# Nobita421/signature-Gan

Measured on AMD Instinct MI355X. Metric: signature images/sec (G+D train step, bs64 64x64 z=100), higher is better.
Workload: dtype f32; 1 GPU; configs[1]: reference conv G/D 64x64x1, z=100, batch 64 per GPU, f32, n_critic=1; global_batch=64, parallelism=dp1

## Files before the change

### include/siggan.h

```cpp
#ifndef SIGGAN_H
#define SIGGAN_H

#include <stddef.h>
#include <stdint.h>

#ifdef __cplusplus
extern "C" {
#endif

#define SIGGAN_ABI_VERSION 4

enum {
    SIGGAN_OK = 0,
    SIGGAN_E_INVALID = -1,
    SIGGAN_E_STATE = -2,
    SIGGAN_E_HIP = -3,
    SIGGAN_E_NOMEM = -4
};

typedef struct siggan_ctx siggan_ctx;

typedef struct siggan_config {
    int32_t device;
    int32_t latent_dim;
// ... 2 lines not shown
    int32_t max_batch;
    float   dropout;
    float   leaky_slope;
    uint64_t seed;
    int32_t dtype;
    float   f16_grad_scale;
    int32_t spectral_norm;
    float   g_leaky_slope;
} siggan_config;
enum { SIGGAN_DTYPE_F32 = 0, SIGGAN_DTYPE_BF16 = 1, SIGGAN_DTYPE_F16 = 2 };

typedef struct siggan_storage {
    float *g_params, *g_grads, *g_exp_avg, *g_exp_avg_sq, *g_adam_steps;
    float *g_bn_running_mean, *g_bn_running_var;
    int64_t *g_bn_batches;
    float *d_params, *d_grads, *d_exp_avg, *d_exp_avg_sq, *d_adam_steps;
    float *d_sn_u, *d_sn_v;
} siggan_storage;

typedef struct siggan_hyper {
    double lr, beta1, beta2, eps;
    float label_smoothing;
    float clip_max_norm;
    float grad_scale;
} siggan_hyper;

enum {
    SIGGAN_M_D_LOSS = 0, SIGGAN_M_D_LOSS_REAL, SIGGAN_M_D_LOSS_FAKE, SIGGAN_M_D_REAL_MEAN,
    SIGGAN_M_D_FAKE_MEAN, SIGGAN_M_D_REAL_ACC, SIGGAN_M_D_FAKE_ACC, SIGGAN_M_D_GRAD_NORM,
    SIGGAN_M_G_LOSS, SIGGAN_M_G_FAKE_MEAN, SIGGAN_M_G_GRAD_NORM,
    SIGGAN_M_D_SKIPPED, SIGGAN_M_G_SKIPPED,
    SIGGAN_M_COUNT = 16
};

int siggan_abi_version(void);
const char *siggan_last_error(void);
int siggan_create(const siggan_config *cfg, siggan_ctx **out);
int siggan_destroy(siggan_ctx *ctx);

int64_t siggan_param_count(const siggan_ctx *ctx, int which);
int32_t siggan_param_tensors(const siggan_ctx *ctx, int which);
int siggan_param_span(const siggan_ctx *ctx, int which, int32_t idx, int64_t *offset, int64_t *numel);
int64_t siggan_bn_count(const siggan_ctx *ctx);
int64_t siggan_sn_count(const siggan_ctx *ctx, int which);
int32_t siggan_bn_layers(const siggan_ctx *ctx);
int64_t siggan_workspace_bytes(const siggan_ctx *ctx);

int siggan_bind(siggan_ctx *ctx, const siggan_storage *st);
int siggan_params_changed(siggan_ctx *ctx);
int siggan_seed(siggan_ctx *ctx, uint64_t seed, uint64_t offset);
int siggan_rng_state(siggan_ctx *ctx, uint64_t *seed, uint64_t *offset);
#define SIGGAN_MODE_GRAPH 1
#define SIGGAN_MODE_OVERLAP 2
int siggan_set_mode(siggan_ctx *ctx, int32_t mode);

enum { SIGGAN_STEP_TRAINER = 0, SIGGAN_STEP_ABLATION = 1 };
int siggan_set_step_variant(siggan_ctx *ctx, int32_t variant);

int siggan_g_forward(siggan_ctx *ctx, const float *z_dev, int32_t batch, int32_t training,
                     float *images_dev, void *stream);

enum { SIGGAN_IS_NEG = 0, SIGGAN_IS_INK_SIGNED = 1, SIGGAN_IS_INK_UNIT = 2, SIGGAN_IS_COUNT = 3 };
int siggan_g_generate_u8(siggan_ctx *ctx, const float *z_dev, int32_t batch, uint8_t *u8_dev,
                         float *images_dev, int32_t *stats_dev, float threshold, void *stream);

int siggan_g_latent_grad(siggan_ctx *ctx, const float *z_dev, int32_t batch, const uint8_t *target_u8_dev,
                         const float *target_f32_dev, float *dz_dev, float *loss_dev, float *images_dev, void *stream);

typedef struct siggan_latent_objective {
    float recon_weight;
    float realism_weight;
    float prior_weight;
} siggan_latent_objective;

int siggan_g_latent_objective_grad(siggan_ctx *ctx, const float *z_dev, int32_t batch, const uint8_t *target_u8_dev,
                                   const float *target_f32_dev, const siggan_latent_objective *w, float *dz_dev,
                                   float *objective_dev, float *terms_dev, float *probs_dev, float *images_dev, void *stream);

int siggan_g_latent_objective_grad_seeded(siggan_ctx *ctx, const float *z_dev, int32_t batch, const uint8_t *target_u8_dev,
        const float *target_f32_dev, const siggan_latent_objective *w, const float *image_grad_dev, float *dz_dev,
        float *objective_dev, float *terms_dev, float *probs_dev, float *images_dev, void *stream);

int siggan_g_param_grad(siggan_ctx *ctx, const float *z_dev, int32_t batch, const uint8_t *target_u8_dev,
                        const float *target_f32_dev, const siggan_latent_objective *w, int32_t first_layer,
                        float *dparams_dev, float *objective_dev, float *terms_dev, float *probs_dev, float *images_dev,
                        void *stream);

int siggan_d_forward(siggan_ctx *ctx, const float *x_dev, int32_t batch, int32_t training,
                     const float *masks_dev, float *probs_dev, float *features_dev, void *stream);

int siggan_d_score_u8(siggan_ctx *ctx, const uint8_t *u8_dev, int32_t batch, int32_t binarize, float *probs_dev,
                      float *x_dev, void *stream);
int siggan_dequant_table(float *table_host);

int siggan_d_step(siggan_ctx *ctx, const float *real_dev, int32_t batch, const float *z_dev,
                  const float *masks_dev, const siggan_hyper *hp, float *metrics_dev,
                  float *metrics_host, void *stream);
int siggan_g_step(siggan_ctx *ctx, int32_t batch, const float *z_dev, const siggan_hyper *hp,
                  float *metrics_dev, float *metrics_host, void *stream);

#define SIGGAN_COMM_ID_BYTES 128
int siggan_comm_unique_id(void *id_out);
int siggan_comm_init(siggan_ctx *ctx, int32_t rank, int32_t world, const void *id);
int siggan_comm_destroy(siggan_ctx *ctx);
int32_t siggan_comm_world(const siggan_ctx *ctx);
int siggan_comm_broadcast(siggan_ctx *ctx, void *buf_dev, int64_t bytes, int32_t root, void *stream);
// ... 45 lines not shown
```

### signature-gan_amd/csrc/gconv.h

```cpp
#pragma once
#include <hip/hip_runtime.h>
#include <stdint.h>
#include <vector>

#include "act.h"

namespace siggan {

enum Epilogue : int {
    EPI_RAW = 0,
    EPI_BIAS_LRELU_DROP,
    EPI_AFFINE_RELU,
    EPI_LRELU_BWD,
    EPI_BN_BWD_STATS,
};

struct GConvArgs {
    int dt;
    const void* in;
    const void* wp;
    void* out;
    int B, Hi, Wi, Ci, Co;
    int lgHr, lgWr;
    int Ho, Wo;
    int form;
    int M;
    int epi;
    const float* bias;
    const float* noise;
    const float* scale;
    const float* shift;
    const void* aref;
    const float* bnp;
    float* stat0;
    float* stat1;
    int64_t stat_cap;
    const float* cls_w;
    float* cls_part;
    float slope;
    float gslope;
    float* slab;
    int64_t slab_floats;
    size_t slab_stride;
    const float* zeros;
};

struct BnBwdParams { f32x4 sc, sf, mu, rs; };
__device__ __forceinline__ BnBwdParams bn_bwd_params(const float* __restrict__ bnp, int Co, int co) {
    BnBwdParams q;
    q.sc = *reinterpret_cast<const f32x4*>(bnp + co); q.sf = *reinterpret_cast<const f32x4*>(bnp + Co + co);
    q.mu = *reinterpret_cast<const f32x4*>(bnp + 2 * Co + co); q.rs = *reinterpret_cast<const f32x4*>(bnp + 3 * Co + co);
    return q;
}
template <class T, bool LK>
__device__ __forceinline__ void bn_bwd_stat_terms(const f32x4 v, const f32x4 y, const BnBwdParams& q, float gs, f32x4& s0, f32x4& s1) {
#pragma unroll
    for (int e = 0; e < 4; ++e) {
        const float vq = (float)(T)v[e];
        const float d = g_dact<LK>(fmaf(y[e], q.sc[e], q.sf[e]), vq, gs);
        s0[e] += d;
        s1[e] = fmaf(d, (y[e] - q.mu[e]) * q.rs[e], s1[e]);
    }
}
__host__ __device__ inline bool gen_lk(const GConvArgs& a) {
    return a.gslope != 0.f && (a.epi == EPI_AFFINE_RELU || a.epi == EPI_BN_BWD_STATS);
}

struct WgradArgs {
    int dt;
    const void* S;
    const void* L;
    float* slab;
    float* dw;
    float* db;
    int B, Cs, Cl;
    int lgHs, lgWs, lgCl;
    int K;
    int kchunk;
    const float* zeros;
};

struct Prof {
    struct Rec {
        int id; double flops, bytes; hipEvent_t e0, e1;
        int form, epi_req, epi, M, Ci, Co;
    };
    static constexpr int NID = 8;
    std::vector<Rec> recs;
    static const char* name(int id);
    void begin(int id, double flops, double bytes, hipStream_t st);
    void shape(const GConvArgs& a, int epi_req);
    void clear();
};
extern Prof* g_prof;

int launch_gconv(const GConvArgs& a, hipStream_t st);
void launch_gconv16(int cfg, const GConvArgs& a, dim3 grid, hipStream_t st, hipEvent_t e0, hipEvent_t e1, int kq = 1);
void launch_wgrad16(bool small, const WgradArgs& a, dim3 grid, hipStream_t st, hipEvent_t e0, hipEvent_t e1);
int launch_wgrad(WgradArgs a, int max_splits, hipStream_t st);

}
```

### signature-gan_amd/csrc/gconv.hip

```cpp
#include "gconv.h"
#include <hip/hip_ext.h>

namespace siggan {


static constexpr int BK = 32;
static constexpr int PAD = 4;

__device__ __forceinline__ int xcd_remap(int bid, int nwg) {
    const int q = nwg >> 3, r = nwg & 7, xcd = bid & 7, idx = bid >> 3;
    return (xcd < r ? xcd * (q + 1) : r * (q + 1) + (xcd - r) * q) + idx;
}

template <int BM, int BN, int WM, int WN, int BK = 32, int DEEP = 0, int KQ = 1, bool LK = false>
__global__ __launch_bounds__(256 * KQ) void k_gconv(const GConvArgs a) {
    constexpr int TM = BM / (32 * WM), TN = BN / (32 * WN);
    constexpr int PA = BM / 32, PB = BN / 32;
    constexpr int KC = BK / 32;
    constexpr int LD = BK + 4;
    __shared__ __attribute__((aligned(16))) float smem[KQ * 2 * LD * (BM + BN)];
    const int quad = KQ > 1 ? (int)(threadIdx.x >> 8) : 0;
    float* const sA = smem + quad * (2 * LD * (BM + BN));
    float* const sB = sA + 2 * LD * BM;

    const int tid = threadIdx.x & 255, lane = tid & 63, wave = tid >> 6;
    const int li = lane & 31, lh = lane >> 5;
    const int wm = wave / WN, wn = wave % WN;
    const float* const a_in = static_cast<const float*>(a.in);
    const float* const a_wp = static_cast<const float*>(a.wp);

    const int tiles_n = a.Co / BN;
    const int bid = xcd_remap(blockIdx.x, gridDim.x);
    const int m0 = (bid / tiles_n) * BM, n0 = (bid % tiles_n) * BN;
    const int cls = blockIdx.z, ph = cls >> 1, pw = cls & 1;
    const int Hr = 1 << a.lgHr, Wr = 1 << a.lgWr;
    const int ntaps = a.form == 0 ? 16 : 4;
    const int Ktot = ntaps * a.Ci;
    const int lgcpt = 31 - __builtin_clz(a.Ci / BK);
    const int nk_all = ntaps << lgcpt;
    const int kper = (nk_all + gridDim.y * KQ - 1) / (gridDim.y * KQ);
    const int k_lo = (blockIdx.y * KQ + quad) * kper;
    const int k_hi = min(nk_all, k_lo + kper);
    const int nk = k_hi - k_lo;

    const int kc = tid & 7, rloc = tid >> 3;
    const float* a_base[PA];
    int a_ih0[PA], a_iw0[PA];
#pragma unroll
    for (int p = 0; p < PA; ++p) {
        const int m = m0 + rloc + 32 * p;
        if (m < a.M) {
            const int n = m >> (a.lgHr + a.lgWr);
            const int rh = (m >> a.lgWr) & (Hr - 1), rw = m & (Wr - 1);
            a_base[p] = a_in + (size_t)n * a.Hi * a.Wi * a.Ci + kc * 4;
            if (a.form == 0) { a_ih0[p] = 2 * rh - 1; a_iw0[p] = 2 * rw - 1; }
            else             { a_ih0[p] = rh + ph;    a_iw0[p] = rw + pw; }
        } else {
            a_base[p] = a_in; a_ih0[p] = -(1 << 20); a_iw0[p] = -(1 << 20);
        }
    }
    const float* wcur = a_wp + ((size_t)cls * a.Co + n0 + rloc) * Ktot + kc * 4 + (size_t)k_lo * BK;

    const float* a_cur[PA];
    int a_step[PA];
    int l_tap = k_lo >> lgcpt, l_cc = k_lo & ((1 << lgcpt) - 1);
    auto set_tap = [&]() __attribute__((always_inline)) {
        int dh, dw;
        if (a.form == 0) { dh = l_tap >> 2; dw = l_tap & 3; } else { dh = -(l_tap >> 1); dw = -(l_tap & 1); }
#pragma unroll
        for (int p = 0; p < PA; ++p) {
            const int ih = a_ih0[p] + dh, iw = a_iw0[p] + dw;
            const bool ok = (unsigned)ih < (unsigned)a.Hi && (unsigned)iw < (unsigned)a.Wi;
            a_cur[p] = ok ? a_base[p] + ((size_t)(ih * a.Wi + iw) * a.Ci + l_cc * BK) : a.zeros;
            a_step[p] = ok ? BK : 0;
        }
    };
    constexpr int NSET = DEEP ? 2 : 1;
    f32x4 ra[NSET][PA][KC], rb[NSET][PB][KC];
    auto load_tile = [&](int set = 0) __attribute__((always_inline)) {
#pragma unroll
        for (int p = 0; p < PA; ++p) {
#pragma unroll
            for (int q = 0; q < KC; ++q) ra[set][p][q] = *reinterpret_cast<const f32x4*>(a_cur[p] + 32 * q);
            a_cur[p] += a_step[p];
        }
#pragma unroll
        for (int p = 0; p < PB; ++p)
#pragma unroll
            for (int q = 0; q < KC; ++q) rb[set][p][q] = *reinterpret_cast<const f32x4*>(wcur + (size_t)(32 * p) * Ktot + 32 * q);
        wcur += BK;
        if (++l_cc == (1 << lgcpt)) { l_cc = 0; ++l_tap; set_tap(); }
    };
    auto store_tile = [&](int buf, int set = 0) __attribute__((always_inline)) {
        float* dA = sA + buf * LD * BM + rloc * LD + kc * 4;
        float* dB = sB + buf * LD * BN + rloc * LD + kc * 4;
#pragma unroll
        for (int p = 0; p < PA; ++p)
#pragma unroll
            for (int q = 0; q < KC; ++q) *reinterpret_cast<f32x4*>(dA + 32 * p * LD + 32 * q) = ra[set][p][q];
#pragma unroll
        for (int p = 0; p < PB; ++p)
#pragma unroll
            for (int q = 0; q < KC; ++q) *reinterpret_cast<f32x4*>(dB + 32 * p * LD + 32 * q) = rb[set][p][q];
    };

    f32x16 acc[TM][TN];
#pragma unroll
    for (int i = 0; i < TM; ++i)
#pragma unroll
        for (int j = 0; j < TN; ++j)
#pragma unroll
            for (int r = 0; r < 16; ++r) acc[i][j][r] = 0.f;

    if (DEEP && nk >= 5) {
        auto tile = [&](const int h, const int kt, const bool st, const bool ld) __attribute__((always_inline)) {
            const float* pA = sA + h * LD * BM + (wm * (32 * TM) + li) * LD + 4 * lh;
            const float* pB = sB + h * LD * BN + (wn * (32 * TN) + li) * LD + 4 * lh;
            f32x4 fa[2][TM], fb[2][TN];
#pragma unroll
            for (int i = 0; i < TM; ++i) fa[0][i] = *reinterpret_cast<const f32x4*>(pA + 32 * i * LD);
#pragma unroll
            for (int j = 0; j < TN; ++j) fb[0][j] = *reinterpret_cast<const f32x4*>(pB + 32 * j * LD);
#pragma unroll
            for (int c = 0; c < BK / 8; ++c) {
                const int cur = c & 1, nxt = cur ^ 1;
                if (c + 1 < BK / 8) {
#pragma unroll
                    for (int i = 0; i < TM; ++i) fa[nxt][i] = *reinterpret_cast<const f32x4*>(pA + 32 * i * LD + 8 * (c + 1));
#pragma unroll
                    for (int j = 0; j < TN; ++j) fb[nxt][j] = *reinterpret_cast<const f32x4*>(pB + 32 * j * LD + 8 * (c + 1));
                }
                __builtin_amdgcn_sched_barrier(0);
#pragma unroll
                for (int t = 0; t < 4; ++t)
#pragma unroll
                    for (int i = 0; i < TM; ++i)
#pragma unroll
                        for (int j = 0; j < TN; ++j)
                            acc[i][j] = __builtin_amdgcn_mfma_f32_32x32x2f32(fa[cur][i][t], fb[cur][j][t], acc[i][j], 0, 0, 0);
                if (c == 0 && st) store_tile(h ^ 1, h ^ 1);
                if (c == 1 && ld) load_tile(h ^ 1);
            }
            __syncthreads();
        };
        set_tap();
        load_tile(0);
        load_tile(1);
        store_tile(0, 0);
        load_tile(0);
        __syncthreads();
        int kt = 0;
        for (; kt + 4 < nk; kt += 2) {
            tile(0, kt, true, true);
            tile(1, kt + 1, true, true);
        }
        for (; kt < nk; kt += 2) {
            tile(0, kt, kt + 1 < nk, kt + 3 < nk);
            if (kt + 1 < nk) tile(1, kt + 1, kt + 2 < nk, kt + 4 < nk);
        }
    } else {
    if (nk > 0) {
        set_tap();
        load_tile();
        store_tile(0);
        if (nk > 1) load_tile();
    }
    __syncthreads();

    for (int kt = 0; kt < nk; ++kt) {
        const int buf = kt & 1;
        const float* pA = sA + buf * LD * BM + (wm * (32 * TM) + li) * LD + 4 * lh;
        const float* pB = sB + buf * LD * BN + (wn * (32 * TN) + li) * LD + 4 * lh;
        f32x4 fa[2][TM], fb[2][TN];
#pragma unroll
        for (int i = 0; i < TM; ++i) fa[0][i] = *reinterpret_cast<const f32x4*>(pA + 32 * i * LD);
#pragma unroll
        for (int j = 0; j < TN; ++j) fb[0][j] = *reinterpret_cast<const f32x4*>(pB + 32 * j * LD);
#pragma unroll
        for (int c = 0; c < BK / 8; ++c) {
            const int cur = c & 1, nxt = cur ^ 1;
            if (c + 1 < BK / 8) {
#pragma unroll
                for (int i = 0; i < TM; ++i) fa[nxt][i] = *reinterpret_cast<const f32x4*>(pA + 32 * i * LD + 8 * (c + 1));
#pragma unroll
                for (int j = 0; j < TN; ++j) fb[nxt][j] = *reinterpret_cast<const f32x4*>(pB + 32 * j * LD + 8 * (c + 1));
            }
            __builtin_amdgcn_sched_barrier(0);
#pragma unroll
            for (int t = 0; t < 4; ++t)
#pragma unroll
                for (int i = 0; i < TM; ++i)
#pragma unroll
                    for (int j = 0; j < TN; ++j)
                        acc[i][j] = __builtin_amdgcn_mfma_f32_32x32x2f32(fa[cur][i][t], fb[cur][j][t], acc[i][j], 0, 0, 0);
            if (c == 0 && kt + 1 < nk) store_tile(buf ^ 1);
            if (c == 1 && kt + 2 < nk) load_tile();
        }
        __syncthreads();
    }
    }

    float* const outp = gridDim.y > 1 ? a.slab + (size_t)blockIdx.y * a.slab_stride : static_cast<float*>(a.out);
    const int epi = gridDim.y > 1 ? (int)EPI_RAW : a.epi;
    constexpr int LDT = BN + 4;
    static_assert(BM * LDT <= 2 * LD * (BM + BN), "output tile must fit the staging buffers");
    float* const sT = smem;
    if (KQ > 1) {
        float* const red = smem + 2 * LD * (BM + BN);
        if (quad == 1) {
#pragma unroll
            for (int i = 0; i < TM; ++i)
#pragma unroll
                for (int j = 0; j < TN; ++j)
#pragma unroll
                    for (int r = 0; r < 16; ++r) red[(((wave * TM + i) * TN + j) * 16 + r) * 64 + lane] = acc[i][j][r];
        }
        __syncthreads();
        if (quad == 0) {
#pragma unroll
            for (int i = 0; i < TM; ++i)
#pragma unroll
                for (int j = 0; j < TN; ++j)
#pragma unroll
                    for (int r = 0; r < 16; ++r) acc[i][j][r] += red[(((wave * TM + i) * TN + j) * 16 + r) * 64 + lane];
        }
    }
    if (quad == 0) {
#pragma unroll
        for (int i = 0; i < TM; ++i)
#pragma unroll
            for (int j = 0; j < TN; ++j)
#pragma unroll
                for (int r = 0; r < 16; ++r)
                    sT[(wm * (32 * TM) + 32 * i + (r & 3) + 8 * (r >> 2) + 4 * lh) * LDT + wn * (32 * TN) + 32 * j + li] = acc[i][j][r];
    }
    __syncthreads();
    if (quad != 0 && epi != EPI_BN_BWD_STATS) return;
    constexpr int C4 = BN / 4, RPP = 256 / C4;
    const int c4 = tid % C4, r0 = tid / C4;
    const int co = n0 + c4 * 4;
    BnBwdParams bq;
    f32x4 st0 = {0.f, 0.f, 0.f, 0.f}, st1 = st0;
    if (epi == EPI_BN_BWD_STATS) bq = bn_bwd_params(a.bnp, a.Co, co);
    const f32x4 bias4 = epi == EPI_BIAS_LRELU_DROP ? *reinterpret_cast<const f32x4*>(a.bias + co) : f32x4{0.f, 0.f, 0.f, 0.f};
    f32x4 sc4 = {1.f, 1.f, 1.f, 1.f}, sh4 = {0.f, 0.f, 0.f, 0.f};
    if (epi == EPI_AFFINE_RELU) { sc4 = *reinterpret_cast<const f32x4*>(a.scale + co); sh4 = *reinterpret_cast<const f32x4*>(a.shift + co); }
    const bool use_noise = (epi == EPI_BIAS_LRELU_DROP || epi == EPI_LRELU_BWD) && a.noise != nullptr;
#pragma unroll
    for (int p = 0; p < BM / RPP; ++p) {
        const int row = r0 + RPP * p, m = m0 + row;
        if (m >= a.M || quad != 0) continue;
        const int n = m >> (a.lgHr + a.lgWr);
        size_t opix;
        if (a.form == 0) {
            opix = (size_t)m;
        } else {
            const int rh = (m >> a.lgWr) & (Hr - 1), rw = m & (Wr - 1);
            opix = ((size_t)n * a.Ho + 2 * rh + ph) * a.Wo + 2 * rw + pw;
        }
        const size_t o = opix * a.Co + co;
        f32x4 v = *reinterpret_cast<const f32x4*>(sT + row * LDT + c4 * 4);
        if (epi == EPI_BN_BWD_STATS) {
            bn_bwd_stat_terms<float, LK>(v, *reinterpret_cast<const f32x4*>(static_cast<const float*>(a.aref) + o), bq, a.gslope, st0, st1);
        } else if (epi == EPI_BIAS_LRELU_DROP) {
#pragma unroll
            for (int e = 0; e < 4; ++e) { float t = v[e] + bias4[e]; v[e] = t > 0.f ? t : t * a.slope; }
            if (use_noise) {
                const f32x4 nz = *reinterpret_cast<const f32x4*>(a.noise + (size_t)n * a.Co + co);
#pragma unroll
                for (int e = 0; e < 4; ++e) v[e] *= nz[e];
            }
        } else if (epi == EPI_AFFINE_RELU) {
#pragma unroll
            for (int e = 0; e < 4; ++e) v[e] = g_act<LK>(fmaf(v[e], sc4[e], sh4[e]), a.gslope);
        } else if (epi == EPI_LRELU_BWD) {
            const f32x4 ar = *reinterpret_cast<const f32x4*>(static_cast<const float*>(a.aref) + o);
#pragma unroll
            for (int e = 0; e < 4; ++e) v[e] *= ar[e] > 0.f ? 1.f : a.slope;
            if (use_noise) {
                const f32x4 nz = *reinterpret_cast<const f32x4*>(a.noise + (size_t)n * a.Co + co);
#pragma unroll
                for (int e = 0; e < 4; ++e) v[e] *= nz[e];
            }
        }
        *reinterpret_cast<f32x4*>(outp + o) = v;
    }
    if (epi == EPI_BN_BWD_STATS) {
        __syncthreads();
        if (quad == 0) {
            *reinterpret_cast<f32x4*>(sT + (size_t)tid * 8) = st0;
            *reinterpret_cast<f32x4*>(sT + (size_t)tid * 8 + 4) = st1;
// ... 172 lines not shown
    if (i >= total4) return;
    const float4* sl = reinterpret_cast<const float4*>(a.slab);
    const size_t stride4 = a.slab_stride / 4;
    float4 v = sl[i];
    for (int z = 1; z < nsplit; ++z) {
        const float4 w = sl[(size_t)z * stride4 + i];
        v.x += w.x; v.y += w.y; v.z += w.z; v.w += w.w;
    }
    const int C4 = a.Co / 4;
    const int64_t per_img = (int64_t)C4 * a.Ho * a.Wo;
    const bool p2 = (C4 & (C4 - 1)) == 0 && (per_img & (per_img - 1)) == 0;
    const int c = (p2 ? (int)(i & (C4 - 1)) : (int)(i % C4)) * 4;
    const int64_t n = p2 ? i >> (63 - __builtin_clzll(per_img)) : i / per_img;
    float* e = reinterpret_cast<float*>(&v);
    if (a.epi == EPI_BIAS_LRELU_DROP) {
#pragma unroll
        for (int k = 0; k < 4; ++k) {
            float x = e[k] + a.bias[c + k];
            x = x > 0.f ? x : x * a.slope;
            if (a.noise) x *= a.noise[n * a.Co + c + k];
            e[k] = x;
        }
    } else if (a.epi == EPI_AFFINE_RELU) {
#pragma unroll
        for (int k = 0; k < 4; ++k) e[k] = g_act<LK>(fmaf(e[k], a.scale[c + k], a.shift[c + k]), a.gslope);
    } else if (a.epi == EPI_LRELU_BWD) {
        const f32x4 ar = ld4<T>(static_cast<const T*>(a.aref) + i * 4);
        const float* r = reinterpret_cast<const float*>(&ar);
#pragma unroll
        for (int k = 0; k < 4; ++k) {
            float x = e[k] * (r[k] > 0.f ? 1.f : a.slope);
            if (a.noise) x *= a.noise[n * a.Co + c + k];
            e[k] = x;
        }
    }
    st4<T>(static_cast<T*>(a.out) + i * 4, f32x4{v.x, v.y, v.z, v.w});
    if (a.cls_w) {
        __shared__ float shc[4];
        const f32x4 w4 = *reinterpret_cast<const f32x4*>(a.cls_w + (size_t)(p2 ? (i & (per_img - 1)) : (i % per_img)) * 4);
        float d = (float)(T)v.x * w4[0];
        d = fmaf((float)(T)v.y, w4[1], d); d = fmaf((float)(T)v.z, w4[2], d); d = fmaf((float)(T)v.w, w4[3], d);
#pragma unroll
        for (int o = 32; o > 0; o >>= 1) d += __shfl_down(d, o, 64);
        if ((threadIdx.x & 63) == 0) shc[threadIdx.x >> 6] = d;
        __syncthreads();
        if (threadIdx.x == 0) a.cls_part[blockIdx.x] = ((shc[0] + shc[1]) + shc[2]) + shc[3];
    }
}

Prof* g_prof = nullptr;

const char* Prof::name(int id) {
    static const char* n[NID] = {"k_gconv<128,128>", "k_gconv<128,64>", "k_gconv<64,64>", "k_gconv<128,32>",
                                 "k_wgrad<64,64>", "k_gconv_up4", "k_wgrad<32,128>", "?"};
    return n[id < 0 || id >= NID ? NID - 1 : id];
}
void Prof::begin(int id, double flops, double bytes, hipStream_t) {
    Rec r; r.id = id; r.flops = flops; r.bytes = bytes;
    r.form = r.epi_req = r.epi = r.M = r.Ci = r.Co = -1;
    (void)hipEventCreate(&r.e0); (void)hipEventCreate(&r.e1);
    recs.push_back(r);
}
void Prof::shape(const GConvArgs& a, int epi_req) {
    Rec& r = recs.back();
    r.form = a.form; r.epi_req = epi_req; r.epi = a.epi; r.M = a.M; r.Ci = a.Ci; r.Co = a.Co;
}
void Prof::clear() {
    for (auto& r : recs) { (void)hipEventDestroy(r.e0); (void)hipEventDestroy(r.e1); }
    recs.clear();
}

static double gconv_bytes(const GConvArgs& a) {
    const double es = (double)dt_size(a.dt);
    const double in = (double)a.B * a.Hi * a.Wi * a.Ci, out = (double)a.B * a.Ho * a.Wo * a.Co, w = 16.0 * a.Ci * a.Co;
    return es * (in + w + out * (a.epi == EPI_LRELU_BWD ? 2.0 : 1.0));
}
static double wgrad_bytes(const WgradArgs& a) {
    const double es = (double)dt_size(a.dt);
    return es * ((double)a.K * a.Cs + 4.0 * a.K * a.Cl) + 4.0 * 16.0 * a.Cs * a.Cl;
}

template <int BM, int BN, int WM, int WN, int BKT = 32, int DEEP = 0, int KQ = 1>
static int launch_cfg(const GConvArgs& a_in, hipStream_t st, int id, int nsplit) {
    GConvArgs a = a_in;
    const int tiles = ((a.M + BM - 1) / BM) * (a.Co / BN);
    const int ncls = a.form == 0 ? 1 : 4;
    const int64_t total4 = (int64_t)a.B * a.Ho * a.Wo * a.Co / 4;
    int rows = 0;
    if (a.epi == EPI_BN_BWD_STATS) {
        if (nsplit > 1 && (256 % (a.Co / 4)) != 0) nsplit = 1;
        rows = nsplit > 1 ? (int)((total4 + 255) / 256) : ((a.M + BM - 1) / BM) * ncls;
        if ((int64_t)2 * rows * a.Co > a.stat_cap) { a.epi = EPI_RAW; rows = 0; }
        else a.stat1 = a.stat0 + (size_t)rows * a.Co;
    }
    if (a.cls_w) {
        const int64_t per_img4 = (int64_t)a.Ho * a.Wo * a.Co / 4;
        if (nsplit > 1 && a.epi != EPI_BN_BWD_STATS && total4 % 256 == 0 && per_img4 % 256 == 0) rows = (int)(per_img4 / 256);
        else a.cls_w = nullptr;
    }
    dim3 grid(tiles, nsplit, ncls);
    if (g_prof) {
        g_prof->begin(id, 2.0 * a.M * a.Co * (double)((a.form == 0 ? 16 : 4) * a.Ci) * ncls, gconv_bytes(a), st);
        g_prof->shape(a, a_in.epi);
    }
    hipEvent_t e0 = g_prof ? g_prof->recs.back().e0 : nullptr, e1 = g_prof ? g_prof->recs.back().e1 : nullptr;
    if (a.dt != DT_F32) {
        launch_gconv16(id, a, grid, st, e0, e1, KQ);
    } else if (gen_lk(a)) {
        hipExtLaunchKernelGGL((k_gconv<BM, BN, WM, WN, BKT, DEEP, KQ, true>), grid, dim3(256 * KQ), 0, st, e0, e1, 0, a);
    } else if (g_prof) {
        hipExtLaunchKernelGGL((k_gconv<BM, BN, WM, WN, BKT, DEEP, KQ>), grid, dim3(256 * KQ), 0, st, e0, e1, 0, a);
    } else {
        hipLaunchKernelGGL((k_gconv<BM, BN, WM, WN, BKT, DEEP, KQ>), grid, dim3(256 * KQ), 0, st, a);
    }
    if (nsplit > 1)
        SIGGAN_GS_SWITCH(gen_lk(a) ? 1.f : 0.f, LK, SIGGAN_DT_SWITCH(a.dt, T, hipLaunchKernelGGL((k_splitk_epilogue<T, LK>),
            dim3((unsigned)((total4 + 255) / 256)), dim3(256), 0, st, a, nsplit, total4)));
    return rows;
}

int launch_gconv(const GConvArgs& a_in, hipStream_t st) {
    GConvArgs a = a_in;
    if (a.epi == EPI_BN_BWD_STATS && (a.stat0 == nullptr || a.stat_cap <= 0)) return -1;
    const int ncls = a.form == 0 ? 1 : 4;
    auto blocks = [&](int bm, int bn) { return ((a.M + bm - 1) / bm) * (a.Co / bn) * ncls; };
    const int nk = (a.form == 0 ? 16 : 4) * (a.Ci / BK);
    auto splits = [&](int nblk) {
        int ns = 1;
        if (a.slab && nblk < 384) {
            ns = (512 + nblk - 1) / nblk;
            if (ns > nk / 4) ns = nk / 4;
            if (ns > 8) ns = 8;
            const int64_t out_floats = (int64_t)a.B * a.Ho * a.Wo * a.Co;
            if (ns > 1 && (int64_t)ns * out_floats > a.slab_floats) ns = (int)(a.slab_floats / out_floats);
            if (ns < 1) ns = 1;
        }
        a.slab_stride = (size_t)a.B * a.Ho * a.Wo * a.Co;
        return ns;
    };
    if (a.Co >= 64) {
        if (a.Co >= 128 && blocks(128, 128) >= 512) return launch_cfg<128, 128, 2, 2, 32, 1>(a, st, 0, 1);
        const int ns = splits(blocks(64, 64));
        if (ns == 2 && (nk & 1) == 0) return launch_cfg<64, 64, 2, 2, 32, 1, 2>(a, st, 2, 1);
        if (ns == 4 && !a.cls_w && a.dt != DT_F32 && (nk & 1) == 0) return launch_cfg<64, 64, 2, 2, 32, 1, 2>(a, st, 2, 1);
        return launch_cfg<64, 64, 2, 2, 32, 1>(a, st, 2, ns);
    }
    if (a.dt == DT_F32 && a.form == 1 && a.Co == 32 && (a.epi == EPI_RAW || a.epi == EPI_AFFINE_RELU) && (a.Ci == 32 || a.Ci == 64) &&
        a.M / 128 >= (a.Ci == 32 ? 384 : 768) && a.M % 128 == 0 &&
        ((1 << (a.lgHr + a.lgWr)) % 128) == 0 && a.lgWr >= 4 && a.lgWr <= 6) {
        dim3 grid(a.M / 128);
        if (g_prof) {
            g_prof->begin(5, 2.0 * a.M * a.Co * (double)(4 * a.Ci) * 4, gconv_bytes(a), st);
            g_prof->shape(a, a.epi);
        }
        hipEvent_t e0 = g_prof ? g_prof->recs.back().e0 : nullptr, e1 = g_prof ? g_prof->recs.back().e1 : nullptr;
        if (gen_lk(a)) {
            if (a.Ci == 32) hipExtLaunchKernelGGL((k_gconv_up4<32, true>), grid, dim3(256), 0, st, e0, e1, 0, a);
            else hipExtLaunchKernelGGL((k_gconv_up4<64, true>), grid, dim3(256), 0, st, e0, e1, 0, a);
        } else {
            if (a.Ci == 32) hipExtLaunchKernelGGL((k_gconv_up4<32, false>), grid, dim3(256), 0, st, e0, e1, 0, a);
            else hipExtLaunchKernelGGL((k_gconv_up4<64, false>), grid, dim3(256), 0, st, e0, e1, 0, a);
        }
        return 0;
    }
    const int ns = splits(blocks(128, 32));
    return launch_cfg<128, 32, 4, 1, 32, 1>(a, st, 3, ns);
}

template <int BM, int BN, int WM, int WN>
__global__ __launch_bounds__(256) void k_wgrad(const WgradArgs a) {
    constexpr int TM = BM / (32 * WM), TN = BN / (32 * WN);
    constexpr int LDA = BM + PAD, LDB = BN + PAD;
    constexpr int CA = BM / 4, RA = 256 / CA, PA = BK / RA;
    constexpr int CB = BN / 4, RB = 256 / CB, PB = BK / RB;
    __shared__ __attribute__((aligned(16))) float smem[2 * BK * (LDA + LDB)];
    float* const sA = smem;
    float* const sB = smem + 2 * BK * LDA;

    const int tid = threadIdx.x, lane = tid & 63, wave = tid >> 6;
    const int li = lane & 31, lh = lane >> 5;
    const int wm = wave / WN, wn = wave % WN;
    const int N = 16 << a.lgCl;
    const int tiles_n = N / BN;
    const int lin = blockIdx.z * gridDim.x + blockIdx.x;
    const int lid = xcd_remap(lin, gridDim.x * gridDim.z);
    const int bx = lid % gridDim.x, bz = lid / gridDim.x;
    const int i0 = (bx / tiles_n) * BM, j0 = (bx % tiles_n) * BN;
    const int kbeg = bz * a.kchunk;
    const int kend = min(a.K, kbeg + a.kchunk);
    const int nk = (kend - kbeg + BK - 1) / BK;
    const int Hs = 1 << a.lgHs, Ws = 1 << a.lgWs, Hl = 2 * Hs, Wl = 2 * Ws, Cl = 1 << a.lgCl;

    const int ca = tid % CA, ka = tid / CA;
    const int cb = tid % CB, kb = tid / CB;
    const float* const a_S = static_cast<const float*>(a.S);
    const float* const a_L = static_cast<const float*>(a.L);
    const int jj = j0 + cb * 4, tap = jj >> a.lgCl, lch = jj & (Cl - 1);
// ... 223 lines not shown
```

### signature-gan_amd/csrc/siggan.hip

```cpp
#include <hip/hip_runtime.h>
#include <dlfcn.h>
#include <math.h>
#include <stdarg.h>
#include <stdio.h>
#include <stdlib.h>
#include <string.h>
#include <new>
#include <vector>

#include "../../include/siggan.h"
#include "gconv.h"
#include "host.h"
#include "ops.h"

using namespace siggan;

static thread_local char g_err[512] = "";
static int fail(int code, const char* fmt, ...) {
    va_list ap;
    va_start(ap, fmt);
    vsnprintf(g_err, sizeof g_err, fmt, ap);
    va_end(ap);
    return code;
}
// ... 614 lines not shown
            if (kind == DV_FC) { j.type = PREP_FC_T; j.O = r.A; j.I = r.Bc; }
            else if (kind == DV_T16) { j.type = PREP_CLS; j.O = r.A; }
            else if (kind == DV_BN) {
                j.type = PREP_BN_EVAL; j.O = r.A; j.perm = r.Bc; j.src2 = P + r.off2;
                j.src3 = c->st.g_bn_running_mean + r.bn_off; j.src4 = c->st.g_bn_running_var + r.bn_off;
            } else {
                if (r.dst2) { PrepJob sc = j; sc.type = PREP_SCALE; sc.O = (int)r.n; sc.dst = r.dst2; prep_add(t, sc); }
                j.type = PREP_TAPS; j.O = r.A; j.I = r.Bc;
            }
            prep_add(t, j);
        }
}
static void repack(const siggan_ctx* c, Lanes& L, hipStream_t sg, hipStream_t sd, bool do_g, bool do_d, int sn_slot = 0, const float* conv1_x = nullptr,
                   int conv1_r0 = 0, int conv1_B = 0) {
    PrepTable t;
    if (do_g) {
        prep_table(c, 0, 0, t);
        if (!launch_prepare(t, BN_EPS, sg)) L.note(hipErrorInvalidValue);
    }
    if (do_d) {
        prep_table(c, 1, sn_slot, t);
        bool ok;
        if (conv1_x && !c->sn) {
            const int64_t H = c->S >> 1;
            char* out = c->d_a[1] + (size_t)((int64_t)conv1_r0 * H * H * c->dC[1]) * c->es;
            ok = launch_prepare_conv1(t, BN_EPS, c->dt, conv1_x, DP(c, di_w(1)), DP(c, di_b(1)), c->cfg.leaky_slope, out, conv1_B, c->S, sd);
        } else {
            ok = launch_prepare(t, BN_EPS, sd);
        }
        if (!ok) L.note(hipErrorInvalidValue);
    }
}
static void ap_table(const siggan_ctx* c, int which, int nride, ApTable& t) {
    t.njobs = 0; t.overflow = 0;
    for (const Derived& r : c->rec[which]) {
        ApJob j; memset(&j, 0, sizeof j);
        j.off = r.off; j.dst = r.dst;
        if (r.kind == DV_FLAT || r.kind == DV_FC) { j.type = AP_FLAT; j.n = r.n + r.n2; ap_add(t, j); continue; }
        j.A = r.A; j.Bc = r.Bc;
        if (r.kind == DV_CONV) { j.type = AP_CONV; j.dt = c->dt; j.dst2 = r.dst2; }
        else if (r.kind == DV_T16) j.type = AP_T16;
        else if (r.kind == DV_BN) {
            j.type = AP_BN; j.off2 = r.off2;
            j.rmean = c->st.g_bn_running_mean + r.bn_off; j.rvar = c->st.g_bn_running_var + r.bn_off;
        } else { j.type = AP_TAPS; j.n = r.n; j.off2 = r.off2; j.n2 = r.n2; j.wait = nride; }
        ap_add(t, j);
    }
}

static GConvArgs gconv_args(const siggan_ctx* c, int form, int B, int h_in, int c_in, int c_out) {
    GConvArgs a; memset(&a, 0, sizeof a);
    a.dt = c->dt; a.gslope = c->cfg.g_leaky_slope;
    a.slab = c->slab_k; a.slab_floats = c->slab_k_floats; a.zeros = c->zeros;
    const int h_small = form == 0 ? h_in / 2 : h_in;
    a.form = form; a.B = B; a.Hi = a.Wi = h_in; a.Ci = c_in; a.Co = c_out;
    a.Ho = a.Wo = form == 0 ? h_in / 2 : 2 * h_in;
    a.lgHr = a.lgWr = ilog2i(h_small); a.M = B * h_small * h_small;
    return a;
}
struct WgradCall { WgradArgs w; int max_splits; };
static WgradCall wgrad_args(const siggan_ctx* c, const void* small, const void* large, float* dw, float* slab, int B, int h_small,
                            int c_small, int c_large) {
    WgradCall g; memset(&g, 0, sizeof g);
    WgradArgs& w = g.w;
    w.zeros = c->zeros; w.dt = c->dt;
    w.S = small; w.L = large; w.slab = slab; w.dw = dw; w.B = B; w.Cs = c_small; w.Cl = c_large;
    w.lgHs = w.lgWs = ilog2i(h_small); w.lgCl = ilog2i(c_large); w.K = B * h_small * h_small;
    g.max_splits = (int)(c->slab_floats / ((int64_t)c_small * (16 * c_large + 1)));
    return g;
}

static int g_forward_pass(const siggan_ctx* c, const float* z, int B, bool training, float* img, hipStream_t s,
                           float* partial = nullptr, float* slab_k = nullptr, uint32_t rng_sid = 0, float* z_out = nullptr,
                           hipEvent_t done = nullptr,
                           uint8_t* u8 = nullptr, int32_t* stats = nullptr, float thr = 0.f,
                           bool keep_y = false) {
    if (!partial) partial = c->partial;
    char* const* const A = training ? c->g_a : c->g_ae;
    const float gs = c->cfg.g_leaky_slope;
    if (c->fc_fused && launch_fc_fwd_fused(c->dt, z, GP(c, gi_fc_w()), GP(c, gi_fc_b()), c->fc_y, A[0], GP(c, gi_bn0_w()),
                                          GP(c, gi_bn0_b()), c->st.g_bn_running_mean, c->st.g_bn_running_var, c->st.g_bn_batches,
                                          c->g_bn[0], training ? nullptr : c->g_bne[0], z_out, c->dev, rng_sid, B, c->latent,
                                          c->gC[0], BN_MOMENTUM, BN_EPS, gs, s)) {
    } else if (!training) {
        launch_fc_fwd(c->dt, z, c->wfc_t, GP(c, gi_fc_b()), A[0], B, c->latent, c->gC[0], gs, s, c->g_bne[0], c->dev, rng_sid, z_out);
    } else {
        launch_fc_fwd(c->dt, z, c->wfc_t, GP(c, gi_fc_b()), c->fc_y, B, c->latent, c->gC[0], gs, s, nullptr, c->dev, rng_sid, z_out);
        launch_bn_train_stats(c->dt, c->fc_y, B, c->F, GP(c, gi_bn0_w()), GP(c, gi_bn0_b()), c->st.g_bn_running_mean,
                              c->st.g_bn_running_var, c->st.g_bn_batches, c->g_bn[0], partial, c->gC[0], BN_MOMENTUM,
                              BN_EPS, s);
        launch_bn_relu(c->dt, c->fc_y, A[0], B, c->F, c->g_bn[0], gs, s);
    }
    for (int l = 1; l <= c->Lg; ++l) {
        const int Hi = 4 << (l - 1), C = c->gC[l];
        GConvArgs a = gconv_args(c, 1, B, Hi, c->gC[l - 1], C);
        if (slab_k) a.slab = slab_k;
        a.in = A[l - 1]; a.wp = c->g_up[l];
        const int64_t off = c->g_bn_off[l];
        if (training) {
            a.out = c->g_y[l]; a.epi = EPI_RAW;
            launch_gconv(a, s);
            const int64_t R = (int64_t)B * 4 * Hi * Hi;
            launch_bn_train_stats(c->dt, c->g_y[l], R, C, GP(c, gi_bn_w(l)), GP(c, gi_bn_b(l)), c->st.g_bn_running_mean + off,
                                  c->st.g_bn_running_var + off, c->st.g_bn_batches + l, c->g_bn[l], partial, 0,
                                  BN_MOMENTUM, BN_EPS, s);
            if (l < c->Lg) launch_bn_relu(c->dt, c->g_y[l], A[l], R, C, c->g_bn[l], gs, s);
// ... 419 lines not shown
    }
    hipEvent_t e_in = c->ev_bridge[0], e_out = c->ev_bridge[1];
    HIPCHK(hipEventRecord(e_in, u));
    HIPCHK(hipStreamWaitEvent(c->s_m, e_in, 0));
    HIPCHK(hipGraphLaunch(exec, c->s_m));
    HIPCHK(hipEventRecord(e_out, c->s_m));
    HIPCHK(hipStreamWaitEvent(u, e_out, 0));
    return SIGGAN_OK;
}
static int run_phase(siggan_ctx* c, const PhaseKey& k, hipStream_t u) {
    PhaseResult r;
    const int rc = enqueue_phase(c, k, u, r);
    Carried& cs = c->cs;
    auto put = [](auto& field, int v) { if (v >= 0) field = v; };
    put(cs.early_ar, r.early_ar); put(cs.dreal_joined, r.dreal_joined); put(cs.dreal_noise2, r.dreal_noise2);
    put(cs.gfwd_joined, r.gfwd_joined); put(cs.g_r0, r.g_r0); put(cs.ga_last_B, r.ga_last_B);
    put(cs.lP[0], r.lP[0]); put(cs.lP[1], r.lP[1]);
    return rc;
}

static PhaseKey make_key(siggan_ctx* c, int phase, int B, bool has_z, bool has_masks, const siggan_hyper* hp,
                         float* metrics_dev) {
    PhaseKey k; memset(&k, 0, sizeof k);
    k.phase = phase; k.B = B; k.has_z = has_z; k.has_masks = has_masks;
    k.mt = metrics_dev ? metrics_dev : c->metrics;
    if (phase <= 1) { k.g_dirty = c->g_dirty; k.d_dirty = c->d_dirty; k.ls = hp->label_smoothing; }
    else {
        k.lr = hp->lr; k.beta1 = hp->beta1; k.beta2 = hp->beta2; k.eps = hp->eps;
        k.clip = hp->clip_max_norm > 0.f ? hp->clip_max_norm : 0.f;
        k.gs = hp->grad_scale > 0.f ? hp->grad_scale : 1.0f;
    }
    return k;
}

static int finish_metrics(siggan_ctx* c, float* metrics_dev, float* metrics_host, hipStream_t s) {
    if (metrics_host) {
        HIPCHK(hipMemcpyAsync(metrics_host, metrics_dev ? metrics_dev : c->metrics, SIGGAN_M_COUNT * sizeof(float),
                              hipMemcpyDeviceToHost, s));
        HIPCHK(hipStreamSynchronize(s));
    }
    return SIGGAN_OK;
}

extern "C" int siggan_set_step_variant(siggan_ctx* c, int32_t variant) {
    if (!c) return fail(SIGGAN_E_INVALID, "null context");
    if (variant != SIGGAN_STEP_TRAINER && variant != SIGGAN_STEP_ABLATION) return fail(SIGGAN_E_INVALID, "unknown step variant %d", variant);
    if (c->cs.g_fwd_pending || c->cs.pending) return fail(SIGGAN_E_STATE, "a step is in flight");
    c->variant = variant;
    return SIGGAN_OK;
}

extern "C" int siggan_set_mode(siggan_ctx* c, int32_t mode) {
    if (!c) return fail(SIGGAN_E_INVALID, "null context");
    c->mode = mode;
    return SIGGAN_OK;
}

static int begin_eval(siggan_ctx* c, hipStream_t s, bool with_d, bool sn_power_iteration) {
    if (with_d) invalidate(c, INV_ROWS);
    const int rc = settle(c, s);
    if (rc) return rc;
    Lanes L(c, s);
    if (with_d) {
        if (c->sn) launch_sn_sigma(c->snt, sn_power_iteration, 2, SN_EPS, s);
        repack(c, L, s, s, c->g_dirty, c->sn || c->d_dirty, 2);
        c->g_dirty = c->d_dirty = false;
    } else {
        repack(c, L, s, s, c->g_dirty, !c->sn && c->d_dirty);
        c->g_dirty = false; if (!c->sn) c->d_dirty = false;
    }
    return SIGGAN_OK;
}

extern "C" int siggan_g_forward(siggan_ctx* c, const float* z_dev, int32_t batch, int32_t training, float* images_dev,
                                void* stream) {
    ENTER(c);
    int rc = check_call(c, batch);
    if (rc) return rc;
    if (training && (rc = check_bn_batch(c, batch))) return rc;
    if (!z_dev || !images_dev) return fail(SIGGAN_E_INVALID, "null tensor");
    hipStream_t s = (hipStream_t)stream;
    if ((rc = begin_eval(c, s, false, false))) return rc;
    c->cs.ga_last_B = g_forward_pass(c, z_dev, batch, training != 0, images_dev, s);
    if (training) c->g_dirty = true;
    LAUNCHCHK();
    return lane_check(c);
}

extern "C" int siggan_g_generate_u8(siggan_ctx* c, const float* z_dev, int32_t batch, uint8_t* u8_dev, float* images_dev,
                                    int32_t* stats_dev, float threshold, void* stream) {
    ENTER(c);
    int rc = check_call(c, batch);
    if (rc) return rc;
    if (!z_dev || !u8_dev) return fail(SIGGAN_E_INVALID, "null tensor");
    if (reinterpret_cast<uintptr_t>(u8_dev) & 3) return fail(SIGGAN_E_INVALID, "u8_dev must be 4-byte aligned");
    if (stats_dev && !isfinite(threshold)) return fail(SIGGAN_E_INVALID, "threshold must be finite");
    hipStream_t s = (hipStream_t)stream;
    if ((rc = begin_eval(c, s, false, false))) return rc;
    c->cs.ga_last_B = g_forward_pass(c, z_dev, batch, false, images_dev, s, nullptr, nullptr, 0, nullptr, nullptr, u8_dev, stats_dev, threshold);
    LAUNCHCHK();
    return lane_check(c);
}

static void objective_seeds(siggan_ctx* c, const float* img, int B, const uint8_t* target_u8_dev, const float* target_f32_dev,
                            float wr, float wd, float* realism, float* probs_dev, hipStream_t s) {
    const int Ld = c->Ld, S = c->S;
// ... 649 lines not shown
```

### signature-gan_amd/engine.py

```python
import ctypes as C
import math

import torch

from . import _lib, layout


def _ptr(t):
    return C.c_void_p(t.data_ptr()) if t is not None else C.c_void_p(0)


def _f32(t, device, what):
    if t is None:
        return None
    if t.device != device:
        raise ValueError(f"{what} must live on {device}, got {t.device}")
    if t.dtype != torch.float32:
        raise ValueError(f"{what} must be float32, got {t.dtype}")
    return t.contiguous()


def check_objective_weights(recon_weight, realism_weight, prior_weight, has_target, want_probs=False, seeded=False):
    w = (float(recon_weight), float(realism_weight), float(prior_weight))
    if any(not math.isfinite(x) or x < 0.0 for x in w):
# ... 100 lines not shown
            return
        if self._comm is not None:
            raise RuntimeError(f"batch {batch} exceeds max_batch {self.max_batch}: a context that holds a communicator "
                               "cannot be re-created on one rank alone; size max_batch for the largest batch up front")
        torch.cuda.synchronize(self.device)
        seed, offset = self.rng_state()
        self.lib.siggan_destroy(self._h)
        self._h = None
        self._staged = None
        self.max_batch = 1 << (int(batch) - 1).bit_length()
        self._create_context()
        self._bind()
        if self._mode != 2:
            _lib.check(self.lib.siggan_set_mode(self._h, self._mode))
        self.seed(seed, offset)

    def views(self, which, arena="params"):
        spans = self.g_spans if which == "g" else self.d_spans
        flat = getattr(self, f"{which}_{arena}")
        return {k: flat[o:o + n].view(shape) for k, (o, n, shape) in spans.items()}

    def sn_views(self):
        out = {}
        for base, (u0, rows, v0, cols) in self.sn_spans.items():
            out[base + "weight_u"] = self.d_sn_u[u0:u0 + rows]
            out[base + "weight_v"] = self.d_sn_v[v0:v0 + cols]
        return out

    def bn_views(self):
        out = {}
        for i, (k, (o, n, shape)) in enumerate(self.bn_spans.items()):
            out[k] = self.g_bn_mean[o:o + n]
            out[k.replace("running_mean", "running_var")] = self.g_bn_var[o:o + n]
            out[k.replace("running_mean", "num_batches_tracked")] = self.g_bn_batches[i]
        return out

    def init_reference(self, seed=0):
        gen = torch.Generator().manual_seed(int(seed))
        for which in ("g", "d"):
            for k, v in self.views(which).items():
                if k.endswith("bias"):
                    v.zero_()
                else:
                    mean = 1.0 if ".1.weight" in k else 0.0
                    v.copy_(torch.empty(v.shape).normal_(mean, 0.02, generator=gen))
            for a in ("grads", "exp_avg", "exp_avg_sq", "adam_steps"):
                getattr(self, f"{which}_{a}").zero_()
        self.g_bn_mean.zero_(); self.g_bn_var.fill_(1.0); self.g_bn_batches.zero_()
        self.params_changed()

    def params_changed(self):
        _lib.check(self.lib.siggan_params_changed(self._h))

    def set_mode(self, graph=False, overlap=True):
        self._mode = (1 if graph else 0) | (2 if overlap else 0)
        _lib.check(self.lib.siggan_set_mode(self._h, self._mode))

    def set_step_variant(self, variant="trainer"):
        v = {"trainer": 0, "ablation": 1}[variant]
        _lib.check(self.lib.siggan_set_step_variant(self._h, v))
        self.step_variant = variant

    def ablation_step(self, real, z=None, masks=None, lr_d=2e-4, lr_g=2e-4, beta1=0.5, beta2=0.999, eps=1e-8,
                      label_smoothing=0.9, sync=True):
        if getattr(self, "step_variant", "trainer") != "ablation":
            raise RuntimeError("call set_step_variant('ablation') first")
        self.d_compute_grads(real, z, masks, label_smoothing, mask_passes=3)
        dm = self.d_apply(lr_d, beta1, beta2, eps, None, 1.0, sync)
        self.g_compute_grads(real.shape[0], label_smoothing=label_smoothing)
        gm = self.g_apply(lr_g, beta1, beta2, eps, None, 1.0, sync)
        if sync:
            dm.update(gm)
        return dm

    def seed(self, seed, offset=0):
        self._seed = int(seed)
        _lib.check(self.lib.siggan_seed(self._h, int(seed), int(offset)))

    def rng_state(self):
        s, o = C.c_uint64(), C.c_uint64()
        _lib.check(self.lib.siggan_rng_state(self._h, C.byref(s), C.byref(o)))
        return int(s.value), int(o.value)

    @staticmethod
    def comm_unique_id():
        buf = C.create_string_buffer(128)
        _lib.check(_lib.load().siggan_comm_unique_id(buf))
        return buf.raw

    def comm_init(self, rank, world, unique_id):
        if len(unique_id) != 128:
            raise ValueError("unique_id must be the 128 bytes of Engine.comm_unique_id()")
        self._comm_id = C.create_string_buffer(bytes(unique_id), 128)
        with torch.cuda.device(self.device):
            _lib.check(self.lib.siggan_comm_init(self._h, int(rank), int(world), self._comm_id))
        self._comm = (int(rank), int(world), bytes(unique_id))

    def comm_destroy(self):
        _lib.check(self.lib.siggan_comm_destroy(self._h))
        self._comm = None

    @property
    def comm_world(self):
        return int(self.lib.siggan_comm_world(self._h))

    def comm_broadcast(self, tensor, root=0):
        if tensor.device != self.device or not tensor.is_contiguous():
            raise ValueError("comm_broadcast needs a contiguous tensor on the engine's device")
# ... 412 lines not shown
```

Baseline: 43750 images/s.

## Add in-block 4-way split-K 32x64 conv config for small generator convs

Result: no change. 43780 images/s, median of 4 (+0.1%).

```diff
diff --git a/include/siggan.h b/include/siggan.h
--- a/include/siggan.h
+++ b/include/siggan.h
@@ -78,6 +78,8 @@
 int siggan_rng_state(siggan_ctx *ctx, uint64_t *seed, uint64_t *offset);
 #define SIGGAN_MODE_GRAPH 1
 #define SIGGAN_MODE_OVERLAP 2
+#define SIGGAN_MODE_SLABS 4
+#define SIGGAN_MODE_SPLITK4 8
 int siggan_set_mode(siggan_ctx *ctx, int32_t mode);
 
 enum { SIGGAN_STEP_TRAINER = 0, SIGGAN_STEP_ABLATION = 1 };
diff --git a/signature-gan_amd/csrc/gconv.h b/signature-gan_amd/csrc/gconv.h
--- a/signature-gan_amd/csrc/gconv.h
+++ b/signature-gan_amd/csrc/gconv.h
@@ -42,6 +42,7 @@
     float* slab;
     int64_t slab_floats;
     size_t slab_stride;
+    int split4;
     const float* zeros;
 };
 
@@ -85,7 +86,7 @@
         int id; double flops, bytes; hipEvent_t e0, e1;
         int form, epi_req, epi, M, Ci, Co;
     };
-    static constexpr int NID = 8;
+    static constexpr int NID = 9;
     std::vector<Rec> recs;
     static const char* name(int id);
     void begin(int id, double flops, double bytes, hipStream_t st);
diff --git a/signature-gan_amd/csrc/gconv.hip b/signature-gan_amd/csrc/gconv.hip
--- a/signature-gan_amd/csrc/gconv.hip
+++ b/signature-gan_amd/csrc/gconv.hip
@@ -13,17 +13,20 @@
 }
 
 template <int BM, int BN, int WM, int WN, int BK = 32, int DEEP = 0, int KQ = 1, bool LK = false>
-__global__ __launch_bounds__(256 * KQ) void k_gconv(const GConvArgs a) {
+__global__ __launch_bounds__(64 * WM * WN * KQ) void k_gconv(const GConvArgs a) {
+    constexpr int NT = 64 * WM * WN;
+    constexpr int RS = NT / 8;
+    constexpr int GS = 2 * (BK + 4) * (BM + BN);
     constexpr int TM = BM / (32 * WM), TN = BN / (32 * WN);
-    constexpr int PA = BM / 32, PB = BN / 32;
+    constexpr int PA = BM / RS, PB = BN / RS;
     constexpr int KC = BK / 32;
     constexpr int LD = BK + 4;
     __shared__ __attribute__((aligned(16))) float smem[KQ * 2 * LD * (BM + BN)];
-    const int quad = KQ > 1 ? (int)(threadIdx.x >> 8) : 0;
-    float* const sA = smem + quad * (2 * LD * (BM + BN));
+    const int quad = KQ > 1 ? (int)(threadIdx.x / NT) : 0;
+    float* const sA = smem + quad * GS;
     float* const sB = sA + 2 * LD * BM;
 
-    const int tid = threadIdx.x & 255, lane = tid & 63, wave = tid >> 6;
+    const int tid = threadIdx.x & (NT - 1), lane = tid & 63, wave = tid >> 6;
     const int li = lane & 31, lh = lane >> 5;
     const int wm = wave / WN, wn = wave % WN;
     const float* const a_in = static_cast<const float*>(a.in);
@@ -48,7 +51,7 @@
     int a_ih0[PA], a_iw0[PA];
 #pragma unroll
     for (int p = 0; p < PA; ++p) {
-        const int m = m0 + rloc + 32 * p;
+        const int m = m0 + rloc + RS * p;
         if (m < a.M) {
             const int n = m >> (a.lgHr + a.lgWr);
             const int rh = (m >> a.lgWr) & (Hr - 1), rw = m & (Wr - 1);
@@ -87,7 +90,7 @@
 #pragma unroll
         for (int p = 0; p < PB; ++p)
 #pragma unroll
-            for (int q = 0; q < KC; ++q) rb[set][p][q] = *reinterpret_cast<const f32x4*>(wcur + (size_t)(32 * p) * Ktot + 32 * q);
+            for (int q = 0; q < KC; ++q) rb[set][p][q] = *reinterpret_cast<const f32x4*>(wcur + (size_t)(RS * p) * Ktot + 32 * q);
         wcur += BK;
         if (++l_cc == (1 << lgcpt)) { l_cc = 0; ++l_tap; set_tap(); }
     };
@@ -97,11 +100,11 @@
 #pragma unroll
         for (int p = 0; p < PA; ++p)
 #pragma unroll
-            for (int q = 0; q < KC; ++q) *reinterpret_cast<f32x4*>(dA + 32 * p * LD + 32 * q) = ra[set][p][q];
+            for (int q = 0; q < KC; ++q) *reinterpret_cast<f32x4*>(dA + RS * p * LD + 32 * q) = ra[set][p][q];
 #pragma unroll
         for (int p = 0; p < PB; ++p)
 #pragma unroll
-            for (int q = 0; q < KC; ++q) *reinterpret_cast<f32x4*>(dB + 32 * p * LD + 32 * q) = rb[set][p][q];
+            for (int q = 0; q < KC; ++q) *reinterpret_cast<f32x4*>(dB + RS * p * LD + 32 * q) = rb[set][p][q];
     };
 
     f32x16 acc[TM][TN];
@@ -203,11 +206,12 @@
     float* const outp = gridDim.y > 1 ? a.slab + (size_t)blockIdx.y * a.slab_stride : static_cast<float*>(a.out);
     const int epi = gridDim.y > 1 ? (int)EPI_RAW : a.epi;
     constexpr int LDT = BN + 4;
-    static_assert(BM * LDT <= 2 * LD * (BM + BN), "output tile must fit the staging buffers");
+    static_assert(BM * LDT <= GS, "output tile must fit the staging buffers");
+    static_assert(NT * TM * TN * 16 <= GS, "a group's accumulators must fit its staging buffers");
     float* const sT = smem;
     if (KQ > 1) {
-        float* const red = smem + 2 * LD * (BM + BN);
-        if (quad == 1) {
+        if (quad != 0) {
+            float* const red = smem + quad * GS;
 #pragma unroll
             for (int i = 0; i < TM; ++i)
 #pragma unroll
@@ -218,11 +222,15 @@
         __syncthreads();
         if (quad == 0) {
 #pragma unroll
-            for (int i = 0; i < TM; ++i)
-#pragma unroll
-                for (int j = 0; j < TN; ++j)
-#pragma unroll
-                    for (int r = 0; r < 16; ++r) acc[i][j][r] += red[(((wave * TM + i) * TN + j) * 16 + r) * 64 + lane];
+            for (int g = 1; g < KQ; ++g) {
+                const float* const red = smem + g * GS;
+#pragma unroll
+                for (int i = 0; i < TM; ++i)
+#pragma unroll
+                    for (int j = 0; j < TN; ++j)
+#pragma unroll
+                        for (int r = 0; r < 16; ++r) acc[i][j][r] += red[(((wave * TM + i) * TN + j) * 16 + r) * 64 + lane];
+            }
         }
     }
     if (quad == 0) {
@@ -236,7 +244,7 @@
     }
     __syncthreads();
     if (quad != 0 && epi != EPI_BN_BWD_STATS) return;
-    constexpr int C4 = BN / 4, RPP = 256 / C4;
+    constexpr int C4 = BN / 4, RPP = NT / C4;
     const int c4 = tid % C4, r0 = tid / C4;
     const int co = n0 + c4 * 4;
     BnBwdParams bq;
@@ -515,7 +523,7 @@
 
 const char* Prof::name(int id) {
     static const char* n[NID] = {"k_gconv<128,128>", "k_gconv<128,64>", "k_gconv<64,64>", "k_gconv<128,32>",
-                                 "k_wgrad<64,64>", "k_gconv_up4", "k_wgrad<32,128>", "?"};
+                                 "k_wgrad<64,64>", "k_gconv_up4", "k_wgrad<32,128>", "k_gconv<32,64>x4", "?"};
     return n[id < 0 || id >= NID ? NID - 1 : id];
 }
 void Prof::begin(int id, double flops, double bytes, hipStream_t) {
@@ -570,11 +578,11 @@
     if (a.dt != DT_F32) {
         launch_gconv16(id, a, grid, st, e0, e1, KQ);
     } else if (gen_lk(a)) {
-        hipExtLaunchKernelGGL((k_gconv<BM, BN, WM, WN, BKT, DEEP, KQ, true>), grid, dim3(256 * KQ), 0, st, e0, e1, 0, a);
+        hipExtLaunchKernelGGL((k_gconv<BM, BN, WM, WN, BKT, DEEP, KQ, true>), grid, dim3(64 * WM * WN * KQ), 0, st, e0, e1, 0, a);
     } else if (g_prof) {
-        hipExtLaunchKernelGGL((k_gconv<BM, BN, WM, WN, BKT, DEEP, KQ>), grid, dim3(256 * KQ), 0, st, e0, e1, 0, a);
+        hipExtLaunchKernelGGL((k_gconv<BM, BN, WM, WN, BKT, DEEP, KQ>), grid, dim3(64 * WM * WN * KQ), 0, st, e0, e1, 0, a);
     } else {
-        hipLaunchKernelGGL((k_gconv<BM, BN, WM, WN, BKT, DEEP, KQ>), grid, dim3(256 * KQ), 0, st, a);
+        hipLaunchKernelGGL((k_gconv<BM, BN, WM, WN, BKT, DEEP, KQ>), grid, dim3(64 * WM * WN * KQ), 0, st, a);
     }
     if (nsplit > 1)
         SIGGAN_GS_SWITCH(gen_lk(a) ? 1.f : 0.f, LK, SIGGAN_DT_SWITCH(a.dt, T, hipLaunchKernelGGL((k_splitk_epilogue<T, LK>),
@@ -588,12 +596,14 @@
     const int ncls = a.form == 0 ? 1 : 4;
     auto blocks = [&](int bm, int bn) { return ((a.M + bm - 1) / bm) * (a.Co / bn) * ncls; };
     const int nk = (a.form == 0 ? 16 : 4) * (a.Ci / BK);
+    int ns_tiles = 1;
     auto splits = [&](int nblk) {
         int ns = 1;
         if (a.slab && nblk < 384) {
             ns = (512 + nblk - 1) / nblk;
             if (ns > nk / 4) ns = nk / 4;
             if (ns > 8) ns = 8;
+            ns_tiles = ns;
             const int64_t out_floats = (int64_t)a.B * a.Ho * a.Wo * a.Co;
             if (ns > 1 && (int64_t)ns * out_floats > a.slab_floats) ns = (int)(a.slab_floats / out_floats);
             if (ns < 1) ns = 1;
@@ -606,6 +616,9 @@
         const int ns = splits(blocks(64, 64));
         if (ns == 2 && (nk & 1) == 0) return launch_cfg<64, 64, 2, 2, 32, 1, 2>(a, st, 2, 1);
         if (ns == 4 && !a.cls_w && a.dt != DT_F32 && (nk & 1) == 0) return launch_cfg<64, 64, 2, 2, 32, 1, 2>(a, st, 2, 1);
+        const bool own_chip = a.form == 1 && a.epi == EPI_AFFINE_RELU;
+        if (a.dt == DT_F32 && ns_tiles == 4 && (nk & 3) == 0 && !a.cls_w && (a.split4 == 2 || (a.split4 == 0 && own_chip)))
+            return launch_cfg<32, 64, 1, 2, 32, 1, 4>(a, st, 7, 1);
         return launch_cfg<64, 64, 2, 2, 32, 1>(a, st, 2, ns);
     }
     if (a.dt == DT_F32 && a.form == 1 && a.Co == 32 && (a.epi == EPI_RAW || a.epi == EPI_AFFINE_RELU) && (a.Ci == 32 || a.Ci == 64) &&
diff --git a/signature-gan_amd/csrc/siggan.hip b/signature-gan_amd/csrc/siggan.hip
--- a/signature-gan_amd/csrc/siggan.hip
+++ b/signature-gan_amd/csrc/siggan.hip
@@ -690,6 +690,7 @@
     GConvArgs a; memset(&a, 0, sizeof a);
     a.dt = c->dt; a.gslope = c->cfg.g_leaky_slope;
     a.slab = c->slab_k; a.slab_floats = c->slab_k_floats; a.zeros = c->zeros;
+    a.split4 = (c->mode & SIGGAN_MODE_SLABS) ? 1 : (c->mode & SIGGAN_MODE_SPLITK4) ? 2 : 0;
     const int h_small = form == 0 ? h_in / 2 : h_in;
     a.form = form; a.B = B; a.Hi = a.Wi = h_in; a.Ci = c_in; a.Co = c_out;
     a.Ho = a.Wo = form == 0 ? h_in / 2 : 2 * h_in;
@@ -1215,6 +1216,12 @@
 
 extern "C" int siggan_set_mode(siggan_ctx* c, int32_t mode) {
     if (!c) return fail(SIGGAN_E_INVALID, "null context");
+    if (((c->mode ^ mode) & (SIGGAN_MODE_SLABS | SIGGAN_MODE_SPLITK4)) != 0 && !c->graphs.empty()) {
+        DevGuard dg_(c->cfg.device); HIPCHK(dg_.err);
+        HIPCHK(hipDeviceSynchronize());
+        for (auto& e : c->graphs) (void)hipGraphExecDestroy(e.exec);
+        c->graphs.clear();
+    }
     c->mode = mode;
     return SIGGAN_OK;
 }
diff --git a/signature-gan_amd/engine.py b/signature-gan_amd/engine.py
--- a/signature-gan_amd/engine.py
+++ b/signature-gan_amd/engine.py
@@ -176,8 +176,8 @@
     def params_changed(self):
         _lib.check(self.lib.siggan_params_changed(self._h))
 
-    def set_mode(self, graph=False, overlap=True):
-        self._mode = (1 if graph else 0) | (2 if overlap else 0)
+    def set_mode(self, graph=False, overlap=True, slabs=False, splitk4=False):
+        self._mode = (1 if graph else 0) | (2 if overlap else 0) | (4 if slabs else 0) | (8 if splitk4 else 0)
         _lib.check(self.lib.siggan_set_mode(self._h, self._mode))
 
     def set_step_variant(self, variant="trainer"):
```
